# ThatRedox/ChunkyClPlugin

Hardware: NVIDIA B200
Metric: path samples/sec (higher is better)
Workload: dtype f32

## Files before the change

### chunkyclplugin_b200/csrc/ccu_device.cuh

```cuda
#pragma once
#include "ccu_math.cuh"

namespace ccu {

#define CCU_ANY_TYPE 0x7FFFFFFE

struct DScene {
    const int *__restrict__ tree;
    int depth;
    const unsigned *__restrict__ top;
    const unsigned *__restrict__ wide;
    int cell_level, top_log2;
    int use_wide;
    const unsigned *__restrict__ air_top;
    const unsigned *__restrict__ air_wide;
    const unsigned *__restrict__ air_bricks;
    int air_cell_level, air_top_log2;
    const int *__restrict__ block_palette;
    int block_palette_len;
    const int *__restrict__ quad_models;
    const int *__restrict__ aabb_models;
    const int *__restrict__ mat_palette;
    const int4 *__restrict__ block_rec;
    const int4 *__restrict__ mat_rec;
    const int4 *__restrict__ quad_rec;
    const int4 *__restrict__ aabb_rec;
    const int *__restrict__ world_bvh;
    const int *__restrict__ actor_bvh;
    const int *__restrict__ trigs;
    int world_bvh_empty, actor_bvh_empty;
    const int4 *__restrict__ world_rec;
    const int4 *__restrict__ actor_rec;
// ... 376 lines not shown
        lvl -= 2;
        e = __ldg(s.wide + (size_t)e * 64 + ((((bx >> lvl) & 3) << 4) | (((by >> lvl) & 3) << 2) | ((bz >> lvl) & 3)));
    }
    level = (e >> 26) & 31;
    unsigned v = e & CCU_WIDE_ANY;
    return v == CCU_WIDE_ANY ? CCU_ANY_TYPE : (int)v;
}

struct March {
    float3 o, d, inv;
    float t;
    float limit;
    int steps;
};

struct MarchStart { float3 inv; float t; int entered; };
static __device__ __noinline__ MarchStart march_begin_core(int depth, float3 origin, float3 direction) {
    MarchStart ms;
    ms.inv = f3(1.0f / direction.x, 1.0f / direction.y, 1.0f / direction.z);
    ms.t = 0;
    ms.entered = 1;
    int lx = f2i(floorf(origin.x)) >> depth, ly = f2i(floorf(origin.y)) >> depth, lz = f2i(floorf(origin.z)) >> depth;
    if ((lx | ly | lz) != 0) {
        float size = (float)(1 << depth);
        Box cube = {0, size, 0, size, 0, size};
        float dist = box_entry(cube, origin, ms.inv);
        if (is_nan(dist) || dist < 0) ms.entered = 0;
        else ms.t += dist + CCU_OFFSET;
    }
    return ms;
}
__device__ __forceinline__ bool march_begin(const DScene &s, March &m, float3 origin, float3 direction, float limit) {
    const MarchStart ms = march_begin_core(s.depth, origin, direction);
    m.o = origin;
    m.d = direction;
    m.inv = ms.inv;
    m.t = ms.t;
    m.limit = limit;
    m.steps = 0;
    return ms.entered != 0;
}

struct Cell {
    float3 pos, q;
    int bx, by, bz;
};
__device__ __forceinline__ Cell march_cell(const March &m) {
    Cell c;
    c.pos = m.o + m.d * m.t;
    c.q = c.pos + m.d * CCU_OFFSET;
    c.bx = f2i(floorf(c.q.x)); c.by = f2i(floorf(c.q.y)); c.bz = f2i(floorf(c.q.z));
    return c;
}
// ... 25 lines not shown
    if (data == 0) {
        march_exit(m, c, level);
        return 0;
    }
    if (march_block(s, m, data, level, surf, hit_t)) {
        hit_block = data;
        hit_node = node;
        hit_cell = c;
        return 1;
    }
    return 0;
}

__device__ __forceinline__ bool octree_intersect_ref(const DScene &s, float3 origin, float3 direction, Record &rec, HitInfo &hi) {
    March m;
    if (!march_begin(s, m, origin, direction, rec.distance)) return false;
    for (;;) {
        float t;
        int block, node;
        Cell cell;
        int r = march_step_ref(s, m, rec.surf, t, block, node, cell);
        if (r == 1) {
            rec.distance = t;
            rec.material = block;
            hi.node = node;
            hi.kind = 1;
            hi.bx = cell.bx; hi.by = cell.by; hi.bz = cell.bz;
            return true;
        }
        if (r == 2) return false;
    }
// ... 196 lines not shown
```

### chunkyclplugin_b200/csrc/ccu_host.h

```cpp
#pragma once
#include <cuda_runtime.h>

#include <algorithm>
#include <cstdint>
#include <cstring>
#include <memory>
#include <mutex>
#include <string>
#include <thread>
#include <utility>
#include <vector>

#include "../../include/chunkycu.h"
#include "ccu_device.cuh"

namespace ccu_host {

int fail(int code, const char *fmt, ...);
const char *last_error();

#define CU(call)                                                                                                          \
    do {                                                                                                                  \
        cudaError_t e_ = (call);                                                                                          \
        if (e_ != cudaSuccess)                                                                                            \
// ... 115 lines not shown
        return fail(rc, "%s", error.c_str());
    }
};

struct SceneInfo {
    int depth = 0, sky_res = 0;
    int world_root = 0, actor_root = 0, use_bvh2 = 0, use_air = 0, air_deep = 0;
    int world_bvh_empty = 1, actor_bvh_empty = 1;
    int cell_level = 0, top_log2 = 0, use_wide = 0, air_cell_level = 4, air_top_log2 = 0;
    int atlas_w = 0, atlas_h = 0, atlas_layers = 0;
    float sky_intensity = 0;
    int sun_host[6] = {0, 0, 0, 0, 0, 0};
    bool have_sun = false, have_atlas = false, have_sky = false;
    float3 su{}, sv{}, sw{};
    float sun_radius_cos = 0;
};

enum SceneArray { OCTREE, BLOCK_PALETTE, QUAD_MODELS, AABB_MODELS, MAT_PALETTE, TRIANGLES, WORLD_BVH, ACTOR_BVH, N_ARRAYS };
struct ArrayDesc {
    const char *setter;
    bool optional;
};
constexpr ArrayDesc ARRAY_DESC[N_ARRAYS] = {
    {"ccu_scene_set_octree", false},      {"ccu_scene_set_block_palette", false}, {"ccu_scene_set_quad_models", true},
    {"ccu_scene_set_aabb_models", true},  {"ccu_scene_set_material_palette", false}, {"ccu_scene_set_triangles", true},
    {"ccu_scene_set_world_bvh", true},    {"ccu_scene_set_actor_bvh", true},
};
struct PackedArray {
    DevBuf<int> dev;
    std::shared_ptr<const std::vector<int>> host;
// ... 47 lines not shown
    size_t accum_floats = 0;
    size_t accum_align = 256;
    int accum_active = 0;
    const float *window_base = nullptr;
    ccu_host::HostBuf<float> pinned;
    ccu_host::SeedRing seeds;
    ccu_host::DevBuf<int> fh_scratch;
    ccu_host::DevBuf<unsigned> work_counter;
    ccu_host::DevBuf<int> bvh_deep;
    int yield_below = 20;
    int q_refill_min = 8;
    int q_march_bias = 4;
    int q_shade_min = 0;
    int q_sticky_min = 0;
    int q_march_warps = 18;
    int window_spp = 0;
    int closed_spp = 0;
    bool target_live = false;
    ccu_render_params params = {256, 5, 13.0f, 0, 0};
    ccu_host::MergeJob merge;

    float last_ms = 0;
    bool timing_pending = false;
    int64_t launches = 0;
};

namespace ccu_host {
int start_readback(ccu_ctx *c, const float *src_dev, size_t lo, size_t hi, cudaStream_t stream);
int merge_readback(ccu_ctx *c, size_t lo, size_t hi, double *sample_buffer, double ds, double dp, double sinv, unsigned max_threads);
int replicate_scene(ccu_ctx *src, ccu_ctx *dst);
// ... 3 lines not shown
```

### chunkyclplugin_b200/csrc/ccu_layout.h

```cpp
#pragma once
#include <algorithm>
#include <cmath>
#include <cstdlib>
#include <cstring>
#include <thread>
#include <unordered_map>
#include <vector>

#include "ccu_device.cuh"
#include "ccu_march.cuh"

namespace {
struct WideLayout {
    std::vector<unsigned> top, wide;
    int cell_level = 0, top_log2 = 0;
    bool ok = true;
};

inline unsigned wide_leaf(int word, int level, bool &ok) {
    long long v = -(long long)word;
    unsigned val;
    if (v == 0x7FFFFFFELL) val = CCU_WIDE_ANY;
    else if (v >= 0 && v < (long long)CCU_WIDE_ANY) val = (unsigned)v;
    else { ok = false; val = 0; }
// ... 192 lines not shown
                const size_t c0 = (size_t)(dim * t / nt) * dim * dim, c1 = (size_t)(dim * (t + 1) / nt) * dim * dim;
                for (size_t c = c0; c < c1; c++)
                    if (!(b.top[c] & CCU_WIDE_LEAF)) b.top[c] += top_off;
                b.wide.insert(b.wide.end(), p.wide.begin(), p.wide.end());
                b.wide_level.insert(b.wide_level.end(), p.wide_level.begin(), p.wide_level.end());
                b.bricks.insert(b.bricks.end(), p.bricks.begin(), p.bricks.end());
            }
            if (b.wide.size() / 64 >= 0x1FFFFFFu || b.bricks.size() / 256 >= 0x7FFFFFu) b.ok = false;
        }
    }
    if (b.wide.empty()) b.wide.assign(64, air_leaf(1, 0));
    if (b.bricks.empty()) b.bricks.assign(256, 0u);
    return b;
}

struct BvhLayout {
    std::vector<int> rec;
    int root = 0;
    bool ok = true;
};
struct BvhStage {
    BvhLayout world, actor;
    std::vector<int> tris;
    std::unordered_map<int, int> leaf_at;
    bool ok = true;
    int leaf(const std::vector<int> &trigs, int prim, bool &valid) {
        auto [at, fresh] = leaf_at.try_emplace(prim, 0);
        if (!fresh) return at->second;
        if (prim < 0 || (size_t)prim >= trigs.size()) { valid = false; return 0; }
        const int count = trigs[(size_t)prim];
// ... 159 lines not shown
```

### chunkyclplugin_b200/csrc/ccu_march.cuh

```cuda
#pragma once
#include "ccu_device.cuh"

namespace ccu {

#define CCU_BRICK_UNIFORM 0xC0000000u

struct LeanRay {
    float3 o, d, inv, doff;
    float t, limit;
    int steps;
    int fmx, fmy, fmz;
};

__device__ __forceinline__ void lean_prepare(LeanRay &r) {
    r.doff = r.d * CCU_OFFSET;
    r.fmx = r.inv.x < 0.0f ? 0 : -1;
    r.fmy = r.inv.y < 0.0f ? 0 : -1;
    r.fmz = r.inv.z < 0.0f ? 0 : -1;
}

__device__ __forceinline__ float lean_exit_axis(int b, int low, int fm, float q, float inv) {
    const int plane = ((b & ~low) | (low & fm)) - fm;
    return fmaxf(((float)plane - q) * inv, -inff_());
}
// ... 56 lines not shown
    const int level = leaf ? ((int)(e << 1)) >> 27 : lvl_brick;
    const int low = (1 << (level & 31)) - 1;
    const float ex = lean_exit_axis(bx, low, r.fmx, q.x, r.inv.x);
    const float ey = lean_exit_axis(by, low, r.fmy, q.y, r.inv.y);
    const float ez = lean_exit_axis(bz, low, r.fmz, q.z, r.inv.z);
    const float tn = r.t + (fminf(ex, fminf(ey, ez)) + CCU_OFFSET);
    const bool adv = active && !fin && level >= 0;
    r.t = adv ? tn : r.t;
    r.steps += adv ? 1 : 0;
    return active ? (fin ? 2 : (level < 0 ? 1 : 0)) : done;
}

template <bool DEEP>
__device__ __forceinline__ bool octree_intersect_lean(const DScene &s, float3 origin, float3 direction, Record &rec, HitInfo &hi) {
    March m;
    if (!march_begin(s, m, origin, direction, rec.distance)) return false;
    LeanRay r;
    r.o = m.o; r.d = m.d; r.inv = m.inv; r.t = m.t; r.limit = m.limit; r.steps = m.steps;
    lean_prepare(r);
    for (;;) {
        const int st = lean_probe<DEEP, false>(s, s.air_top, r);
        if (st == 0) continue;
        if (st == 2) return false;
        m.t = r.t; m.steps = r.steps;
        const Cell c = march_cell(m);
        int level;
        const int data = find_leaf_wide(s, c.bx, c.by, c.bz, level);
        float t;
        if (march_block(s, m, data, level, rec.surf, t)) {
            rec.distance = t;
            rec.material = data;
// ... 79 lines not shown
```

### chunkyclplugin_b200/csrc/ccu_queue.cuh

```cuda
#pragma once
#include "ccu_march.cuh"

#ifndef CCU_Q_WARPS
#define CCU_Q_WARPS 28
#endif
#ifndef CCU_Q_ROWS
#define CCU_Q_ROWS 32
#endif

namespace ccu {

constexpr int Q_WARPS = CCU_Q_WARPS;
constexpr int Q_ROWS = CCU_Q_ROWS;
constexpr int Q_SLOTS = Q_ROWS * 32;
constexpr int Q_MW = (Q_ROWS + 31) / 32;
static_assert(Q_ROWS >= 1 && Q_ROWS <= 64, "at most two mask words per stage and column");

enum QStage : int { QS_MARCH = 0, QS_BLOCK, QS_EXIT, QS_END, QS_BVH, QS_SHADE, QS_LEAF, QS_COUNT_BVH };
constexpr int QS_COUNT = QS_BVH;

enum QField : int {
    QF_GID = 0, QF_META, QF_RNG, QF_COLX, QF_COLY, QF_COLZ, QF_THRX, QF_THRY, QF_THRZ,
    QF_SNX, QF_SNY, QF_SNZ, QF_SHW,
    QF_OX, QF_OY, QF_OZ, QF_DX, QF_DY, QF_DZ, QF_IX, QF_IY, QF_IZ, QF_T, QF_LIMIT, QF_STEPS,
// ... 172 lines not shown
        }
        do {
            if (LAY != 2) done = lean_step_flat<LAY == 0>(s, top, r, cur >= 0 && done == 0, done);
            else if (cur >= 0 && done == 0) done = lean_probe<LAY == 2, LAY == 0>(s, top, r);
            n_fly = __popc(__ballot_sync(full, cur >= 0 && done == 0));
            QSTAT(10, 1); QSTAT(11, n_fly);
        } while (busy - n_fly < refill_min && n_fly != 0);
    }
    if (cur >= 0) {
        F[QF_T * Q_SLOTS + cur] = __float_as_uint(r.t);
        F[QF_STEPS * Q_SLOTS + cur] = (uint32_t)r.steps;
        q_push(mask, done == 0 ? QS_MARCH : (done == 1 ? QS_BLOCK : QS_EXIT), cur & 31, cur >> 5);
    }
}

__device__ __forceinline__ void q_shade(const DScene &s, uint32_t *F, unsigned *mask, int lane, int row, float3 o, float3 d, float distance,
                                        bool ray_hit, const Surf &hit) {
    const int slot = row * 32 + lane;
    uint32_t meta = QU(QF_META) & ~QM_HIT;
    const bool shadow = (meta & QM_SHADOW) != 0;
    bool sun = false, bounce = false;
    float3 from = o;
    float3 normal = f3(0, 0, 0);
    if (!ray_hit) {
        float3 throughput = f3(QFL(QF_THRX), QFL(QF_THRY), QFL(QF_THRZ));
        float3 color = f3(QFL(QF_COLX), QFL(QF_COLY), QFL(QF_COLZ));
        float3 sky = sky_radiance(s, d);
        color = color + (sky * throughput) * (shadow ? QFL(QF_SHW) : 1.0f);
        QFL(QF_COLX) = color.x; QFL(QF_COLY) = color.y; QFL(QF_COLZ) = color.z;
        if (shadow) bounce = true;
// ... 33 lines not shown
        next_limit = distance;
    } else {
        next_d = diffuse_direction_sc(normal, x1, sn, cs);
        next_o = from + next_d * CCU_OFFSET;
        next_limit = inff_();
        const int ray_depth = (int)((meta >> 16) & 0xFF) + 1;
        meta = (meta & ~(0xFFu << 16) & ~QM_SHADOW) | ((uint32_t)ray_depth << 16);
        QU(QF_META) = meta;
        if (!(ray_depth < s.max_depth)) {
            next_ray = false;
            q_push(mask, QS_END, lane, row);
        }
    }
    if (next_ray) {
        March m;
        const bool entered = march_begin(s, m, next_o, next_d, next_limit);
        q_store_ray(F, mask, lane, row, m, entered);
    }
}

template <bool HAS_BVH>
__device__ __forceinline__ bool q_stage_resolve(const DScene &s, uint32_t *F, unsigned *mask, int lane, const bool kind_block, int min_lanes) {
    const int row = q_pop_batch(mask, kind_block ? QS_BLOCK : QS_EXIT, lane, min_lanes);
    if (row == -2) return false;
    QSTAT(2 * (kind_block ? QS_BLOCK : QS_EXIT), 1); QSTAT(2 * (kind_block ? QS_BLOCK : QS_EXIT) + 1, __popc(__ballot_sync(0xffffffffu, row >= 0)));
    if (row < 0) return true;
    const int slot = row * 32 + lane;
    March m;
    m.o = f3(QFL(QF_OX), QFL(QF_OY), QFL(QF_OZ));
    m.d = f3(QFL(QF_DX), QFL(QF_DY), QFL(QF_DZ));
    m.inv = f3(QFL(QF_IX), QFL(QF_IY), QFL(QF_IZ));
// ... 22 lines not shown
            QFL(QF_HNX) = hit.normal.x; QFL(QF_HNY) = hit.normal.y; QFL(QF_HNZ) = hit.normal.z;
            QFL(QF_HCX) = hit.color.x; QFL(QF_HCY) = hit.color.y; QFL(QF_HCZ) = hit.color.z;
        }
        const uint32_t meta = QU(QF_META);
        QU(QF_META) = ray_hit ? (meta | QM_HIT) : (meta & ~QM_HIT);
        if (ray_hit && (meta & QM_SHADOW)) {
            q_push(mask, QS_SHADE, lane, row);
            return true;
        }
        int ref, phase;
        bvh_first_ref(s, ref, phase);
        QI(QF_BREF) = ref;
        QI(QF_BSP) = phase << 8;
        q_push(mask, ref < 0 ? QS_LEAF : QS_BVH, lane, row);
    } else {
        q_shade(s, F, mask, lane, row, m.o, m.d, distance, ray_hit, hit);
    }
    return true;
}

__device__ __forceinline__ bool q_stage_shade(const DScene &s, uint32_t *F, unsigned *mask, int lane, int min_lanes) {
    const int row = q_pop_batch(mask, QS_SHADE, lane, min_lanes);
    if (row == -2) return false;
    QSTAT(22, 1); QSTAT(23, __popc(__ballot_sync(0xffffffffu, row >= 0)));
    if (row < 0) return true;
    const int slot = row * 32 + lane;
    const float3 o = f3(QFL(QF_OX), QFL(QF_OY), QFL(QF_OZ));
    const float3 d = f3(QFL(QF_DX), QFL(QF_DY), QFL(QF_DZ));
    const bool ray_hit = (QU(QF_META) & QM_HIT) != 0;
    Surf hit;
    hit.normal = f3(QFL(QF_HNX), QFL(QF_HNY), QFL(QF_HNZ));
    hit.color = make_float4(QFL(QF_HCX), QFL(QF_HCY), QFL(QF_HCZ), 0.0f);
    hit.emittance = QFL(QF_HEM);
    q_shade(s, F, mask, lane, row, o, d, QFL(QF_HDIST), ray_hit, hit);
    return true;
}

__device__ __forceinline__ float triangle_hit_aligned(const Int8 &q0, const int *__restrict__ t, float distance, float3 origin, float3 dir, float3 &normal,
                                                      float &ou, float &ov, int &material) {
    const int flags = q0.v[0];
    const float3 e1 = f3(i2f(q0.v[1]), i2f(q0.v[2]), i2f(q0.v[3]));
    const float3 e2 = f3(i2f(q0.v[4]), i2f(q0.v[5]), i2f(q0.v[6]));
    float3 pvec = cross3(dir, e2);
    float det = dot3(e1, pvec);
    if ((flags >> 8) & 1) {
        if (det > -CCU_EPS && det < CCU_EPS) return nanf_();
    } else if (det > -CCU_EPS) {
        return nanf_();
    }
// ... 192 lines not shown
    }
    if (PATCH && tw == Q_TILE_W && bh == Q_TILE_H) {
        ix = (in & 7u) | (((in >> 5) & 3u) << 3);
        iy = ((in >> 3) & 3u) | ((in >> 7) << 2);
    }
    py = band * Q_TILE_H + iy;
    px = tile * Q_TILE_W + ix;
}
template <bool PATCH = false>
__device__ __forceinline__ int tile_order_pixel(unsigned k, int W, int H) {
    unsigned px, py;
    tile_order_xy<PATCH>(k, W, H, px, py);
    return (int)(py * (unsigned)W + px);
}

template <bool LAST_FIRST>
__device__ __forceinline__ bool q_stage_end(const DScene &s, const PassParams &w, uint32_t *F, unsigned *mask, int *live, int lane, int min_lanes) {
    const unsigned full = 0xffffffffu;
    const int row = q_pop_batch(mask, QS_END, lane, min_lanes);
    if (row == -2) return false;
    QSTAT(2 * QS_END, 1); QSTAT(2 * QS_END + 1, __popc(__ballot_sync(full, row >= 0)));
    const int slot = row < 0 ? lane : row * 32 + lane;
    uint32_t meta = row >= 0 ? QU(QF_META) : 0u;
    int gid = row >= 0 ? QI(QF_GID) : 0;
    int pass = (int)(meta & 0xFFFFu);
    bool need_pixel = row >= 0 && (meta & QM_NEEDPIX) != 0;
    if (row >= 0 && !need_pixel) {
        float *px = w.res + (size_t)gid * 3;
        int spp = w.start_spp + pass;
        const float *pr = spp == 0 ? w.res_prev + (size_t)gid * 3 : px;
        float3 mean = f3(__ldcg(pr), __ldcg(pr + 1), __ldcg(pr + 2));
// ... 45 lines not shown
        }
    }
    const unsigned died = __ballot_sync(full, row >= 0 && !alive);
    if (died && lane == (__ffs((int)died) - 1)) atomicSub(live, __popc(died));
    if (!alive) return true;
    QI(QF_GID) = gid;
    QU(QF_META) = (uint32_t)pass;
    QFL(QF_COLX) = 0.0f; QFL(QF_COLY) = 0.0f; QFL(QF_COLZ) = 0.0f;
    QFL(QF_THRX) = 1.0f; QFL(QF_THRY) = 1.0f; QFL(QF_THRZ) = 1.0f;
    uint32_t rng = (uint32_t)__ldg(w.seeds + pass) + (uint32_t)gid;
    rng_next(rng);
    float3 o, d;
    camera_ray<false>(s, gid, rng, o, d);
    QU(QF_RNG) = rng;
    March m;
    const bool entered = march_begin(s, m, o, d, inff_());
    q_store_ray(F, mask, lane, row, m, entered);
    return true;
}

template <bool HAS_BVH, int LAY>
__global__ void __launch_bounds__(Q_WARPS * 32, 1) k_render_queue(const __grid_constant__ DScene s, const __grid_constant__ QueueParams qp) {
    constexpr int NST = q_stages(HAS_BVH);
    constexpr int MASK_WORDS = q_mask_words(HAS_BVH);
    extern __shared__ uint32_t q_mem[];
    uint32_t *F = q_mem;
    unsigned *mask = q_mem + q_fields(HAS_BVH) * Q_SLOTS;
    int *live = reinterpret_cast<int *>(mask + MASK_WORDS);
    unsigned *top_s = mask + MASK_WORDS + 32;
    int *stk = reinterpret_cast<int *>(top_s + (LAY == 0 ? Q_TOP_WORDS : 0));
    const unsigned full = 0xffffffffu;
// ... 47 lines not shown
            if (n > best_n) { best_n = n; best = st; }
        }
        }
        if (best < 0) {
            if (*reinterpret_cast<volatile int *>(live) == 0) break;
            QSTAT(12, 1);
            __nanosleep(100);
            continue;
        }
        const int min_lanes = held < 2 ? qp.shade_min : 1;
        bool ran = true;
        switch (best) {
            case QS_MARCH: QSTAT(0, 1); q_stage_march<NST, LAY>(s, top, F, mask, lane, qp.yield_below, qp.refill_min); break;
            case QS_BLOCK:
            case QS_EXIT: ran = q_stage_resolve<HAS_BVH>(s, F, mask, lane, best == QS_BLOCK, min_lanes); break;
            case QS_END: ran = q_stage_end<!HAS_BVH>(s, qp.w, F, mask, live, lane, min_lanes); break;
            case QS_BVH: QSTAT(16, 1); if (HAS_BVH) q_stage_bvh<NST>(s, F, mask, stk, qp.bvh_deep, lane, qp.yield_below, qp.refill_min); break;
            case QS_LEAF: if (HAS_BVH) ran = q_stage_leaf(s, F, mask, stk, qp.bvh_deep, lane, min_lanes); break;
            default: if (HAS_BVH) ran = q_stage_shade(s, F, mask, lane, min_lanes); break;
        }
        sticky = (ran && best != QS_MARCH && best != QS_BVH) ? best : -1;
        if (ran) {
            held = 0;
        } else {
            held++;
            __nanosleep(40);
        }
        __syncwarp();
    }
}

// ... 6 lines not shown
```

### chunkyclplugin_b200/csrc/chunkycu.cu

```cuda
#include <cuda_runtime.h>

#include <algorithm>
#include <cmath>
#include <cstdarg>
#include <cstdio>
#include <cstdlib>
#include <cstring>
#include <climits>
#include <mutex>
#include <string>
#include <thread>
#include <vector>

#include <chrono>

#include "ccu_host.h"
#include "ccu_march.cuh"
#include "ccu_queue.cuh"
#include "ccu_tonemap.cuh"
#include "ccu_layout.h"

using namespace ccu;


// ... 85 lines not shown
    uint32_t rng = (uint32_t)seed + (uint32_t)gid;
    rng_next(rng);
    float3 o, d;
    camera_ray_xy<false>(s, gid, (int)px, (int)py, rng, o, d);
    if (MODE == 0) {
        Record rec;
        rec.distance = inff_(); rec.material = 0; rec.surf.normal = f3(0, 0, 0); rec.point = f3(0, 0, 0);
        rec.surf.color = make_float4(0, 0, 0, 0); rec.surf.emittance = 0;
        HitInfo hi = {-1, 0, 0, 0, 0};
        bool hit = false;
        if (valid) hit = HAS_BVH ? closest_intersect_ref(s, o, d, rec, hi) : octree_intersect_ref(s, o, d, rec, hi);
        if (valid) first_hit_store(out, gid, hit, rec.material, rec.surf.normal, hi.node, hi.kind, rec.distance, rec.surf.color);
        return;
    }
    March m;
    const bool entered = march_begin(s, m, o, d, inff_());
    LeanRay r;
    r.o = m.o; r.d = m.d; r.inv = m.inv; r.t = m.t; r.limit = m.limit; r.steps = m.steps;
    lean_prepare(r);
    int st = (valid && entered) ? 0 : 2;
    Surf surf;
    surf.normal = f3(0, 0, 0); surf.color = make_float4(0, 0, 0, 0); surf.emittance = 0;
    float distance = inff_();
    int material = 0, hbx = 0, hby = 0, hbz = 0;
    for (;;) {
        st = first_hit_march<MODE == 2>(s, &r, st);
        if (st == 1) {
            m.t = r.t; m.steps = r.steps;
            const Cell c = march_cell(m);
            int level;
            const int data = find_leaf_wide(s, c.bx, c.by, c.bz, level);
// ... 142 lines not shown

int air_layout_id(const ccu_ctx *c) {
    if (c->scene.info.air_deep) return 2;
    return (c->scene.air_top.n <= (size_t)Q_TOP_WORDS && getenv("CCU_NO_TOPS") == nullptr) ? 0 : 1;
}

void fill_view(ccu_host::Scene &sc) {
    DScene &s = sc.view;
    const ccu_host::SceneInfo &in = sc.info;
    const auto arr = [&](ccu_host::SceneArray a) { return (const int *)sc.arrays[a].dev.p; };
    const auto rec = [](const DevBuf<int> &b) { return reinterpret_cast<const int4 *>(b.p); };
    s.tree = arr(ccu_host::OCTREE); s.depth = in.depth;
    s.top = sc.top.p; s.wide = sc.wide.p; s.cell_level = in.cell_level; s.top_log2 = in.top_log2; s.use_wide = in.use_wide;
    s.air_top = sc.air_top.p; s.air_wide = sc.air_wide.p; s.air_bricks = sc.air_bricks.p;
    s.air_cell_level = in.air_cell_level; s.air_top_log2 = in.air_top_log2;
    s.world_rec = rec(sc.world_rec); s.actor_rec = rec(sc.actor_rec); s.tris2 = sc.tris2.p;
    s.world_root = in.world_root; s.actor_root = in.actor_root;
    s.block_palette = arr(ccu_host::BLOCK_PALETTE); s.block_palette_len = (int)sc.arrays[ccu_host::BLOCK_PALETTE].dev.n;
    s.quad_models = arr(ccu_host::QUAD_MODELS); s.aabb_models = arr(ccu_host::AABB_MODELS); s.mat_palette = arr(ccu_host::MAT_PALETTE);
    s.block_rec = rec(sc.block_rec); s.mat_rec = rec(sc.mat_rec); s.quad_rec = rec(sc.quad_rec); s.aabb_rec = rec(sc.aabb_rec);
    s.world_bvh = arr(ccu_host::WORLD_BVH); s.actor_bvh = arr(ccu_host::ACTOR_BVH); s.trigs = arr(ccu_host::TRIANGLES);
    s.world_bvh_empty = in.world_bvh_empty; s.actor_bvh_empty = in.actor_bvh_empty;
    s.atlas = sc.atlas.p;
    s.atlas_w = in.atlas_w; s.atlas_h = in.atlas_h; s.atlas_layers = in.atlas_layers;
    s.atlas_tiles_x = (in.atlas_w + 15) / 16; s.atlas_tiles_y = (in.atlas_h + 15) / 16;
    s.sky = sc.sky.p; s.sky_res = in.sky_res; s.sky_intensity = in.sky_intensity;
    s.su = in.su; s.sv = in.sv; s.sw = in.sw; s.sun_radius_cos = in.sun_radius_cos;
    s.sun_flags = in.sun_host[0]; s.sun_tex_size = in.sun_host[1]; s.sun_tex = in.sun_host[2];
    memcpy(&s.sun_intensity, &in.sun_host[3], 4);
}

DScene launch_view(const ccu_ctx *c) {
    DScene s = c->scene.view;
    if (c->params.flags & CCU_RENDER_NO_ENTITIES) s.world_bvh_empty = s.actor_bvh_empty = 1;
    if (c->params.flags & CCU_RENDER_NO_SUN) s.sun_flags &= ~1;
    s.unorm = c->unorm.p;
    s.projector_type = c->projector_type;
    memcpy(s.cam, c->cam, sizeof s.cam);
    s.rays = c->rays[c->rays_active].p;
    s.width = c->width; s.height = c->height;
    s.half_width = (float)(c->width / (2.0 * c->height));
    s.inv_height = (float)(1.0 / c->height);
    s.draw_depth = c->params.draw_depth; s.max_depth = c->params.max_depth; s.emitter_scale = c->params.emitter_scale;
    return s;
// ... 193 lines not shown
    if (rc != CCU_OK) return rc;
    if (n == 0) return fail(CCU_ENODEVICE, "no CUDA device");
    if (device_index < 0 || device_index >= n) return fail(CCU_EINVAL, "device index %d out of range [0,%d)", device_index, n);
    cudaDeviceProp p;
    CU(cudaGetDeviceProperties(&p, device_index));
    if (p.major != 10) return fail(CCU_ENODEVICE, "device %d is sm_%d%d; this library is built for sm_100a only", device_index, p.major, p.minor);
    ccu_ctx *c = new ccu_ctx();
    c->device = device_index;
    c->sm_count = p.multiProcessorCount;
    if (const char *e = getenv("CCU_Q_MARCH_WARPS")) c->q_march_warps = std::max(1, std::min(64, atoi(e)));
    if (const char *e = getenv("CCU_Q_MARCH_BIAS")) c->q_march_bias = std::max(-32, std::min(32, atoi(e)));
    if (const char *e = getenv("CCU_Q_REFILL_MIN")) c->q_refill_min = std::max(1, std::min(32, atoi(e)));
    if (const char *e = getenv("CCU_Q_STICKY")) c->q_sticky_min = std::max(1, std::min(33, atoi(e)));
    if (const char *e = getenv("CCU_Q_SHADE_MIN")) c->q_shade_min = std::max(0, std::min(32, atoi(e)));
    if (const char *e = getenv("CCU_YIELD_BELOW")) c->yield_below = std::max(0, std::min(33, atoi(e)));
    DeviceGuard g(device_index);
    cudaError_t e = c->stream.create();
    if (e == cudaSuccess) e = c->copy_stream.create();
    if (e == cudaSuccess) e = c->ev0.create(cudaEventDefault);
    if (e == cudaSuccess) e = c->ev1.create(cudaEventDefault);
    if (e == cudaSuccess) e = c->window_ev.create(cudaEventDisableTiming);
    for (Event &ev : c->chunk_ev) if (e == cudaSuccess) e = ev.create(cudaEventDisableTiming);
    for (Event &ev : c->rays_used) if (e == cudaSuccess) e = ev.create(cudaEventDisableTiming);
    for (bool bvh : {false, true})
        for (int lay = 0; lay < 3 && e == cudaSuccess; lay++)
            e = cudaFuncSetAttribute(queue_kernel(bvh, lay), cudaFuncAttributeMaxDynamicSharedMemorySize, Q_SMEM_LIMIT);
    if (e == cudaSuccess) e = c->unorm.alloc(256);
    if (e == cudaSuccess) {
        k_unorm_table<<<1, 256, 0, c->stream>>>(c->unorm.p);
        c->launches++;
// ... 141 lines not shown
        const std::vector<int> &tree = host(ccu_host::OCTREE);
        WideLayout wl = build_wide_layout(tree.data(), tree.size(), in.depth);
        in.use_wide = (enable && wl.ok) ? 1 : 0;
        in.cell_level = wl.cell_level;
        in.top_log2 = wl.top_log2;
        CU(sc.top.upload(wl.top.data(), wl.top.size(), c->stream));
        CU(sc.wide.upload(wl.wide.data(), wl.wide.size(), c->stream));
        AirLayout al = build_air_layout(tree.data(), tree.size(), in.depth);
        in.use_air = (enable && al.ok) ? 1 : 0;
        in.air_cell_level = al.cell_level;
        in.air_top_log2 = al.top_log2;
        in.air_deep = al.cell_level > 4 ? 1 : 0;
        CU(sc.air_top.upload(al.top.data(), al.top.size(), c->stream));
        CU(sc.air_wide.upload(al.wide.data(), al.wide.size(), c->stream));
        CU(sc.air_bricks.upload(al.bricks.data(), al.bricks.size(), c->stream));
    }
    {
        PaletteRecs pr = build_palette_recs(host(ccu_host::BLOCK_PALETTE), host(ccu_host::MAT_PALETTE), host(ccu_host::QUAD_MODELS),
                                            host(ccu_host::AABB_MODELS));
        CU(sc.block_rec.upload(pr.block.data(), pr.block.size(), c->stream));
        CU(sc.mat_rec.upload(pr.mat.data(), pr.mat.size(), c->stream));
        CU(sc.quad_rec.upload(pr.quad.data(), pr.quad.size(), c->stream));
        CU(sc.aabb_rec.upload(pr.aabb.data(), pr.aabb.size(), c->stream));
    }
    {
        const std::vector<int> &world = host(ccu_host::WORLD_BVH), &actor = host(ccu_host::ACTOR_BVH);
        const BvhStage bs = build_bvh_stage(world, actor, host(ccu_host::TRIANGLES));
        in.world_bvh_empty = bvh_is_empty(world);
        in.actor_bvh_empty = bvh_is_empty(actor);
        in.use_bvh2 = bs.ok ? 1 : 0;
// ... 128 lines not shown
static int render_passes_locked(ccu_ctx *c, const int32_t *seeds, int32_t n_passes, bool first_chunk) {
    ccu_host::SeedRing &ring = c->seeds;
    if (!ring.dev.p) {
        ccu_host::SeedRing r;
        CU(r.dev.alloc((size_t)SEED_SLOTS * SEED_SLOT_INTS));
        CU(r.pinned.alloc((size_t)SEED_SLOTS * SEED_SLOT_INTS));
        for (Event &ev : r.ev) CU(ev.create(cudaEventDisableTiming));
        ring = std::move(r);
    }
    const int slot = ring.slot;
    ring.slot = (slot + 1) % SEED_SLOTS;
    CU(cudaEventSynchronize(ring.ev[slot]));
    int *seeds_host = ring.pinned + (size_t)slot * SEED_SLOT_INTS, *seeds_dev = ring.dev.p + (size_t)slot * SEED_SLOT_INTS;
    memcpy(seeds_host, seeds, (size_t)n_passes * sizeof(int));
    CU(cudaMemcpyAsync(seeds_dev, seeds_host, (size_t)n_passes * sizeof(int), cudaMemcpyHostToDevice, c->stream));
    const DScene s = launch_view(c);
    const int n_pixels = c->width * c->height;
    if (!c->work_counter.p) CU(c->work_counter.alloc(1));
    if (first_chunk) CU(cudaEventRecord(c->ev0, c->stream));
    const bool bvh = !(s.world_bvh_empty && s.actor_bvh_empty);
    const int mode = layout_mode(c);
    float *res = c->accum[c->accum_active].p;
    const float *res_prev = c->window_spp == 0 ? c->window_base : res;
    int kernel = c->params.kernel;
    if (kernel == 0) kernel = (mode != 0 && (!bvh || c->scene.info.use_bvh2)) ? 4 : 1;
    if (kernel == 1) {
        const int threads = 128, blocks = (n_pixels + threads - 1) / threads;
        dispatch<3>(mode, [&](auto M) {
            k_render_mega<M><<<blocks, threads, 0, c->stream>>>(s, seeds_dev, n_passes, c->window_spp, res, res_prev, n_pixels);
        });
    } else {
// ... 4 lines not shown
        qp.w.seeds = seeds_dev;
        qp.w.n_passes = n_passes;
        qp.w.start_spp = c->window_spp;
        qp.w.res = res;
        qp.w.res_prev = res_prev;
        qp.w.n_pixels = n_pixels;
        qp.w.next_pixel = c->work_counter.p;
        qp.yield_below = c->yield_below;
        qp.refill_min = c->q_refill_min;
        qp.march_bias = c->q_march_bias;
        qp.shade_min = c->q_shade_min;
        qp.sticky_min = c->q_sticky_min > 0 ? c->q_sticky_min : (bvh ? 16 : 33);
        qp.march_warps = bvh ? 64 : c->q_march_warps;
        const int lay = air_layout_id(c);
        const int grid = c->sm_count, block = Q_WARPS * 32;
        const int sky_texels = c->scene.info.sky_res * c->scene.info.sky_res;
        const int base_smem = q_smem_bytes(bvh, lay == 0);
        const char *sky_env = getenv("CCU_SKY_SMEM_MAX");
        const int sky_max = sky_env ? atoi(sky_env) : 16384;
        const bool sky_smem = sky_texels * 4 <= sky_max && base_smem + sky_texels * 4 <= Q_SMEM_LIMIT;
        qp.sky_texels = sky_smem ? sky_texels : 0;
        qp.bvh_deep = nullptr;
        if (bvh) {
            if (!c->bvh_deep.p) CU(c->bvh_deep.alloc((size_t)c->sm_count * Q_SLOTS * Q_DEEP));
            qp.bvh_deep = c->bvh_deep.p;
        }
        const int smem = base_smem + qp.sky_texels * 4;
        queue_kernel(bvh, lay)<<<grid, block, smem, c->stream>>>(s, qp);
#ifdef CCU_Q_STATS
        {
// ... 365 lines not shown
        return fail(CCU_EINVAL, "ccu_debug_bvh_layout: bad argument");
    const BvhStage s = build_bvh_stage(std::vector<int>(bvh, bvh + n_bvh), {}, std::vector<int>(trigs, trigs + n_trigs));
    const std::vector<int> &r = s.world.rec, &t = s.tris;
    *ok = s.ok ? 1 : 0;
    *root = s.world.root;
    *rec_words = (int64_t)r.size();
    *tris_words = (int64_t)t.size();
    if (rec) {
        if (rec_cap < (int64_t)r.size()) return fail(CCU_EINVAL, "ccu_debug_bvh_layout: rec buffer too small");
        std::copy(r.begin(), r.end(), rec);
    }
    if (tris) {
        if (tris_cap < (int64_t)t.size()) return fail(CCU_EINVAL, "ccu_debug_bvh_layout: tris buffer too small");
        std::copy(t.begin(), t.end(), tris);
    }
    return CCU_OK;
}

int ccu_debug_layout_lookup(const int32_t *tree, int64_t n, int32_t depth, const int32_t *xyz, int64_t count, int32_t *wide_value,
                            int32_t *wide_level, int32_t *air_solid, int32_t *air_level) {
    if (!tree || n < 1 || depth < 0 || depth > 30 || (count > 0 && !xyz)) return fail(CCU_EINVAL, "ccu_debug_layout_lookup: bad argument");
    WideLayout wl = build_wide_layout(tree, (size_t)n, depth);
    AirLayout al = build_air_layout(tree, (size_t)n, depth);
    if (!al.ok) return fail(CCU_ESTATE, "air layout could not be built");
    const int cl = wl.cell_level, tl = wl.top_log2;
    for (int64_t i = 0; i < count; i++) {
        const int bx = xyz[3 * i], by = xyz[3 * i + 1], bz = xyz[3 * i + 2];
        if (((bx | by | bz) >> depth) != 0) return fail(CCU_EINVAL, "voxel %lld outside the octree cube", (long long)i);
        if (wl.ok) {
            const size_t cell = ((((size_t)(bx >> cl) << tl) + (size_t)(by >> cl)) << tl) + (size_t)(bz >> cl);
// ... 37 lines not shown
```

### chunkyclplugin_b200/native.py

```python
from __future__ import annotations

import ctypes as C
import os
from typing import Optional

import numpy as np

_HERE = os.path.dirname(os.path.abspath(__file__))
LIB_PATH = os.environ.get("CHUNKYCU_LIB") or os.path.join(_HERE, "libchunkycu.so")

CCU_RENDER_NO_ENTITIES, CCU_RENDER_NO_SUN = 1, 2
CCU_UNIQUE_ID_BYTES = 128

CCU_OK, CCU_ENODEVICE, CCU_EINVAL, CCU_ECUDA, CCU_ENOMEM, CCU_ESTATE = 0, -1, -2, -3, -4, -5


class ChunkyCuError(RuntimeError):

    def __init__(self, code: int, message: str):
        super().__init__(f"[{code}] {message}")
        self.code = code


class RenderParams(C.Structure):
# ... 39 lines not shown
    "ccu_render_reset_window": (C.c_int, [_vp]),
    "ccu_render_set_window_spp": (C.c_int, [_vp, _i32]),
    "ccu_render_end": (C.c_int, [_vp]),
    "ccu_render_device_buffer": (C.c_int, [_vp, C.POINTER(_vp), C.POINTER(_i64)]),
    "ccu_render_scale": (C.c_int, [_vp, _f]),
    "ccu_stream_handle": (C.c_int, [_vp, C.POINTER(_vp)]),
    "ccu_first_hit": (C.c_int, [_vp, _i32, _vp, _vp, _vp, _vp, _vp, _vp, _vp]),
    "ccu_preview": (C.c_int, [_vp, _vp]),
    "ccu_last_kernel_ms": (C.c_int, [_vp, C.POINTER(_f)]),
    "ccu_launch_count": (C.c_int, [_vp, C.POINTER(_i64)]),
    "ccu_scene_device_bytes": (C.c_int, [_vp, C.POINTER(_i64)]),
    "ccu_scene_commit_ms": (C.c_int, [_vp, C.POINTER(C.c_double)]),
    "ccu_tonemap": (C.c_int, [_vp, _i32, _i32, _f, _vp, _i32, _vp]),
    "ccu_bench_gather": (C.c_int, [_vp, _i64, _i32, C.POINTER(_f), C.POINTER(_f)]),
    "ccu_debug_layout_lookup": (C.c_int, [_vp, _i64, _i32, _vp, _i64, _vp, _vp, _vp, _vp]),
    "ccu_debug_bvh_layout": (C.c_int, [_vp, _i64, _vp, _i64, _vp, _i64, _vp, _i64, C.POINTER(_i64), C.POINTER(_i64), _pi32, _pi32]),
    "ccu_group_create": (C.c_int, [_vp, _i32, C.POINTER(_vp)]),
    "ccu_group_unique_id": (C.c_int, [_vp]),
    "ccu_group_join": (C.c_int, [_vp, _vp, _i32, _i32, C.POINTER(_vp)]),
    "ccu_group_destroy": (C.c_int, [_vp]),
    "ccu_group_size": (C.c_int, [_vp, _pi32, _pi32]),
    "ccu_group_member": (C.c_int, [_vp, _i32, C.POINTER(_vp)]),
    "ccu_group_replicate_scene": (C.c_int, [_vp]),
    "ccu_group_camera_set": (C.c_int, [_vp, _i32, _vp, _i64]),
    "ccu_group_render_begin": (C.c_int, [_vp, _i32, _i32]),
    "ccu_group_render_set_params": (C.c_int, [_vp, C.POINTER(RenderParams)]),
    "ccu_group_render_passes": (C.c_int, [_vp, _vp, _i32]),
    "ccu_group_render_sync": (C.c_int, [_vp]),
    "ccu_group_render_merge": (C.c_int, [_vp, _vp, _i32, _pi32]),
    "ccu_group_render_merge_async": (C.c_int, [_vp, _vp, _i32, _pi32]),
# ... 43 lines not shown

def _ptr(a: Optional[np.ndarray]):
    return None if a is None else a.ctypes.data_as(C.c_void_p)


def layout_lookup(tree: np.ndarray, depth: int, xyz: np.ndarray):
    tree = np.ascontiguousarray(tree, dtype=np.int32)
    xyz = np.ascontiguousarray(xyz, dtype=np.int32).reshape(-1, 3)
    n = xyz.shape[0]
    out = {k: np.empty(n, dtype=np.int32) for k in ("wide_value", "wide_level", "air_solid", "air_level")}
    check(load().ccu_debug_layout_lookup(_ptr(tree), tree.size, depth, _ptr(xyz), n, _ptr(out["wide_value"]), _ptr(out["wide_level"]),
                                         _ptr(out["air_solid"]), _ptr(out["air_level"])))
    return out


def debug_bvh_layout(bvh: np.ndarray, trigs: np.ndarray):
    bvh = np.ascontiguousarray(bvh, dtype=np.int32)
    trigs = np.ascontiguousarray(trigs, dtype=np.int32)
    nr, nt, root, ok = _i64(), _i64(), _i32(), _i32()
    lib = load()
    check(lib.ccu_debug_bvh_layout(_ptr(bvh), bvh.size, _ptr(trigs), trigs.size, None, 0, None, 0, C.byref(nr), C.byref(nt), C.byref(root), C.byref(ok)))
    rec = np.zeros(max(nr.value, 1), dtype=np.int32)
    tris = np.zeros(max(nt.value, 1), dtype=np.int32)
    check(lib.ccu_debug_bvh_layout(_ptr(bvh), bvh.size, _ptr(trigs), trigs.size, _ptr(rec), rec.size, _ptr(tris), tris.size,
                                   C.byref(nr), C.byref(nt), C.byref(root), C.byref(ok)))
    return rec[:nr.value].reshape(-1, 16), tris[:nt.value], root.value, bool(ok.value)


def device_count() -> int:
    n = C.c_int()
# ... 310 lines not shown
```

### include/chunkycu.h

```cpp
#ifndef CHUNKYCU_H
#define CHUNKYCU_H

#include <stddef.h>
#include <stdint.h>

#ifdef __cplusplus
extern "C" {
#endif

#define CCU_OK 0
#define CCU_ENODEVICE (-1)
#define CCU_EINVAL (-2)
#define CCU_ECUDA (-3)
#define CCU_ENOMEM (-4)
#define CCU_ESTATE (-5)

typedef struct ccu_ctx ccu_ctx;

typedef struct ccu_render_params {
    int32_t draw_depth;
    int32_t max_depth;
    float emitter_scale;
    int32_t kernel;
    int32_t flags;
// ... 48 lines not shown

int ccu_first_hit(ccu_ctx *ctx, int32_t seed, int32_t *block, int32_t *face, int32_t *node, int32_t *kind, float *t,
                  float *normal, float *color);

int ccu_preview(ccu_ctx *ctx, int32_t *argb);

int ccu_tonemap(ccu_ctx *ctx, int32_t width, int32_t height, float exposure, const double *input, int32_t type, int32_t *argb);

int ccu_last_kernel_ms(ccu_ctx *ctx, float *ms);
int ccu_launch_count(ccu_ctx *ctx, int64_t *launches);
int ccu_scene_device_bytes(ccu_ctx *ctx, int64_t *bytes);
int ccu_scene_commit_ms(ccu_ctx *ctx, double *ms);
int ccu_bench_gather(ccu_ctx *ctx, int64_t array_bytes, int32_t dependent, float *gbytes_per_s, float *ns_per_load);
int ccu_debug_layout_lookup(const int32_t *tree, int64_t n, int32_t depth, const int32_t *xyz, int64_t count, int32_t *wide_value,
                            int32_t *wide_level, int32_t *air_solid, int32_t *air_level);

int ccu_debug_bvh_layout(const int32_t *bvh, int64_t n_bvh, const int32_t *trigs, int64_t n_trigs, int32_t *rec, int64_t rec_cap,
                         int32_t *tris, int64_t tris_cap, int64_t *rec_words, int64_t *tris_words, int32_t *root, int32_t *ok);

typedef struct ccu_group ccu_group;
#define CCU_UNIQUE_ID_BYTES 128
int ccu_group_create(const int32_t *devices, int32_t n, ccu_group **out);
int ccu_group_unique_id(uint8_t id[CCU_UNIQUE_ID_BYTES]);
int ccu_group_join(ccu_ctx *ctx, const uint8_t id[CCU_UNIQUE_ID_BYTES], int32_t rank, int32_t world, ccu_group **out);
int ccu_group_destroy(ccu_group *g);
int ccu_group_size(ccu_group *g, int32_t *world, int32_t *local_members);
int ccu_group_member(ccu_group *g, int32_t local_index, ccu_ctx **ctx);
int ccu_group_replicate_scene(ccu_group *g);
int ccu_group_camera_set(ccu_group *g, int32_t projector_type, const float *settings, int64_t n_floats);
int ccu_group_render_begin(ccu_group *g, int32_t width, int32_t height);
// ... 15 lines not shown
```

Measured before the change: 3.165 billion.

## Clip octree march limit to bounding box of non-empty voxels

Computes on the host a tight bounding box of all non-air octree nodes, padded by one voxel. At march start, each ray's limit is clipped to where it leaves this box, so rays stop marching through empty space outside the solid region. The clip applies to camera rays and to secondary rays in scenes without a BVH, and only when the box is at most a quarter of the octree volume. It adds a slab test per ray and a host tree walk at scene commit, and it relies on the limit clip being exact near boundaries.

```diff
diff --git a/chunkyclplugin_b200/csrc/ccu_device.cuh b/chunkyclplugin_b200/csrc/ccu_device.cuh
--- a/chunkyclplugin_b200/csrc/ccu_device.cuh
+++ b/chunkyclplugin_b200/csrc/ccu_device.cuh
@@ -16,6 +16,8 @@
     const unsigned *__restrict__ air_wide;
     const unsigned *__restrict__ air_bricks;
     int air_cell_level, air_top_log2;
+    float3 cut_lo, cut_hi;
+    float cut_reach;
     const int *__restrict__ block_palette;
     int block_palette_len;
     const int *__restrict__ quad_models;
@@ -422,8 +424,9 @@
     int steps;
 };
 
-struct MarchStart { float3 inv; float t; int entered; };
-static __device__ __noinline__ MarchStart march_begin_core(int depth, float3 origin, float3 direction) {
+struct MarchStart { float3 inv; float t, limit; int entered; };
+static __device__ __noinline__ MarchStart march_begin_core(int depth, float3 origin, float3 direction, float limit, float3 lo, float3 hi,
+                                                           float reach) {
     MarchStart ms;
     ms.inv = f3(1.0f / direction.x, 1.0f / direction.y, 1.0f / direction.z);
     ms.t = 0;
@@ -436,15 +439,28 @@
         if (is_nan(dist) || dist < 0) ms.entered = 0;
         else ms.t += dist + CCU_OFFSET;
     }
+    ms.limit = limit;
+    if (reach < 0.0f) return ms;
+    const float span = fabsf(origin.x) + fabsf(origin.y) + fabsf(origin.z) + fabsf(direction.x) + fabsf(direction.y) + fabsf(direction.z);
+    const float imax = fmaxf(fabsf(ms.inv.x), fmaxf(fabsf(ms.inv.y), fabsf(ms.inv.z)));
+    if (span <= reach && imax <= 0x1p64f) {
+        const float3 inv = ms.inv;
+        const float nx = ((inv.x >= 0.0f ? lo.x : hi.x) - origin.x) * inv.x, fx = ((inv.x >= 0.0f ? hi.x : lo.x) - origin.x) * inv.x;
+        const float ny = ((inv.y >= 0.0f ? lo.y : hi.y) - origin.y) * inv.y, fy = ((inv.y >= 0.0f ? hi.y : lo.y) - origin.y) * inv.y;
+        const float nz = ((inv.z >= 0.0f ? lo.z : hi.z) - origin.z) * inv.z, fz = ((inv.z >= 0.0f ? hi.z : lo.z) - origin.z) * inv.z;
+        const float enter = fmaxf(nx, fmaxf(ny, nz)), leave = fminf(fx, fminf(fy, fz));
+        ms.limit = fminf(limit, enter > leave ? -inff_() : leave);
+    }
     return ms;
 }
+template <bool CUT>
 __device__ __forceinline__ bool march_begin(const DScene &s, March &m, float3 origin, float3 direction, float limit) {
-    const MarchStart ms = march_begin_core(s.depth, origin, direction);
+    const MarchStart ms = march_begin_core(s.depth, origin, direction, limit, s.cut_lo, s.cut_hi, CUT ? s.cut_reach : -1.0f);
     m.o = origin;
     m.d = direction;
     m.inv = ms.inv;
     m.t = ms.t;
-    m.limit = limit;
+    m.limit = CUT ? ms.limit : limit;
     m.steps = 0;
     return ms.entered != 0;
 }
@@ -500,7 +516,7 @@
 
 __device__ __forceinline__ bool octree_intersect_ref(const DScene &s, float3 origin, float3 direction, Record &rec, HitInfo &hi) {
     March m;
-    if (!march_begin(s, m, origin, direction, rec.distance)) return false;
+    if (!march_begin<true>(s, m, origin, direction, rec.distance)) return false;
     for (;;) {
         float t;
         int block, node;
diff --git a/chunkyclplugin_b200/csrc/ccu_host.h b/chunkyclplugin_b200/csrc/ccu_host.h
--- a/chunkyclplugin_b200/csrc/ccu_host.h
+++ b/chunkyclplugin_b200/csrc/ccu_host.h
@@ -153,6 +153,7 @@
     bool have_sun = false, have_atlas = false, have_sky = false;
     float3 su{}, sv{}, sw{};
     float sun_radius_cos = 0;
+    int solid_lo[3] = {0, 0, 0}, solid_hi[3] = {0, 0, 0};
 };
 
 enum SceneArray { OCTREE, BLOCK_PALETTE, QUAD_MODELS, AABB_MODELS, MAT_PALETTE, TRIANGLES, WORLD_BVH, ACTOR_BVH, N_ARRAYS };
@@ -230,6 +231,7 @@
     int q_shade_min = 0;
     int q_sticky_min = 0;
     int q_march_warps = 18;
+    bool cube_cut = false;
     int window_spp = 0;
     int closed_spp = 0;
     bool target_live = false;
diff --git a/chunkyclplugin_b200/csrc/ccu_layout.h b/chunkyclplugin_b200/csrc/ccu_layout.h
--- a/chunkyclplugin_b200/csrc/ccu_layout.h
+++ b/chunkyclplugin_b200/csrc/ccu_layout.h
@@ -1,5 +1,6 @@
 #pragma once
 #include <algorithm>
+#include <climits>
 #include <cmath>
 #include <cstdlib>
 #include <cstring>
@@ -230,6 +231,45 @@
     return b;
 }
 
+struct SolidBox {
+    int lo[3] = {INT_MAX, INT_MAX, INT_MAX}, hi[3] = {INT_MIN, INT_MIN, INT_MIN};
+    size_t visits = 0;
+    bool covers(int x, int y, int z, int size) const {
+        return x >= lo[0] && y >= lo[1] && z >= lo[2] && x + size <= hi[0] && y + size <= hi[1] && z + size <= hi[2];
+    }
+    void add(int x, int y, int z, int size) {
+        const int p[3] = {x, y, z};
+        for (int i = 0; i < 3; i++) {
+            lo[i] = std::min(lo[i], p[i]);
+            hi[i] = std::max(hi[i], p[i] + size);
+        }
+    }
+};
+
+inline void solid_box_walk(const int *tree, size_t n, size_t idx, int level, int x, int y, int z, SolidBox &b) {
+    const int size = 1 << level;
+    const int w = tree[idx];
+    if (w == 0 || b.visits > n || b.covers(x, y, z, size)) return;
+    b.visits++;
+    if (w < 0 || level == 0 || (size_t)w + 7 >= n) { b.add(x, y, z, size); return; }
+    const int h = level - 1;
+    for (int c = 0; c < 8; c++)
+        solid_box_walk(tree, n, (size_t)w + c, h, x + (((c >> 2) & 1) << h), y + (((c >> 1) & 1) << h), z + ((c & 1) << h), b);
+}
+
+inline SolidBox solid_box(const int *tree, size_t n, int depth) {
+    SolidBox b;
+    solid_box_walk(tree, n, 0, depth, 0, 0, 0, b);
+    if (b.visits > n) {
+        b = SolidBox();
+        b.add(0, 0, 0, 1 << depth);
+    } else if (b.lo[0] > b.hi[0]) {
+        b = SolidBox();
+        for (int i = 0; i < 3; i++) b.lo[i] = b.hi[i] = 0;
+    }
+    return b;
+}
+
 struct BvhLayout {
     std::vector<int> rec;
     int root = 0;
diff --git a/chunkyclplugin_b200/csrc/ccu_march.cuh b/chunkyclplugin_b200/csrc/ccu_march.cuh
--- a/chunkyclplugin_b200/csrc/ccu_march.cuh
+++ b/chunkyclplugin_b200/csrc/ccu_march.cuh
@@ -94,7 +94,7 @@
 template <bool DEEP>
 __device__ __forceinline__ bool octree_intersect_lean(const DScene &s, float3 origin, float3 direction, Record &rec, HitInfo &hi) {
     March m;
-    if (!march_begin(s, m, origin, direction, rec.distance)) return false;
+    if (!march_begin<true>(s, m, origin, direction, rec.distance)) return false;
     LeanRay r;
     r.o = m.o; r.d = m.d; r.inv = m.inv; r.t = m.t; r.limit = m.limit; r.steps = m.steps;
     lean_prepare(r);
diff --git a/chunkyclplugin_b200/csrc/ccu_queue.cuh b/chunkyclplugin_b200/csrc/ccu_queue.cuh
--- a/chunkyclplugin_b200/csrc/ccu_queue.cuh
+++ b/chunkyclplugin_b200/csrc/ccu_queue.cuh
@@ -210,6 +210,7 @@
     }
 }
 
+template <bool HAS_BVH>
 __device__ __forceinline__ void q_shade(const DScene &s, uint32_t *F, unsigned *mask, int lane, int row, float3 o, float3 d, float distance,
                                         bool ray_hit, const Surf &hit) {
     const int slot = row * 32 + lane;
@@ -273,7 +274,7 @@
     }
     if (next_ray) {
         March m;
-        const bool entered = march_begin(s, m, next_o, next_d, next_limit);
+        const bool entered = march_begin<!HAS_BVH>(s, m, next_o, next_d, next_limit);
         q_store_ray(F, mask, lane, row, m, entered);
     }
 }
@@ -326,7 +327,7 @@
         QI(QF_BSP) = phase << 8;
         q_push(mask, ref < 0 ? QS_LEAF : QS_BVH, lane, row);
     } else {
-        q_shade(s, F, mask, lane, row, m.o, m.d, distance, ray_hit, hit);
+        q_shade<false>(s, F, mask, lane, row, m.o, m.d, distance, ray_hit, hit);
     }
     return true;
 }
@@ -344,7 +345,7 @@
     hit.normal = f3(QFL(QF_HNX), QFL(QF_HNY), QFL(QF_HNZ));
     hit.color = make_float4(QFL(QF_HCX), QFL(QF_HCY), QFL(QF_HCZ), 0.0f);
     hit.emittance = QFL(QF_HEM);
-    q_shade(s, F, mask, lane, row, o, d, QFL(QF_HDIST), ray_hit, hit);
+    q_shade<true>(s, F, mask, lane, row, o, d, QFL(QF_HDIST), ray_hit, hit);
     return true;
 }
 
@@ -567,7 +568,7 @@
     return (int)(py * (unsigned)W + px);
 }
 
-template <bool LAST_FIRST>
+template <bool LAST_FIRST, bool CUT>
 __device__ __forceinline__ bool q_stage_end(const DScene &s, const PassParams &w, uint32_t *F, unsigned *mask, int *live, int lane, int min_lanes) {
     const unsigned full = 0xffffffffu;
     const int row = q_pop_batch(mask, QS_END, lane, min_lanes);
@@ -643,7 +644,7 @@
     camera_ray<false>(s, gid, rng, o, d);
     QU(QF_RNG) = rng;
     March m;
-    const bool entered = march_begin(s, m, o, d, inff_());
+    const bool entered = march_begin<CUT>(s, m, o, d, inff_());
     q_store_ray(F, mask, lane, row, m, entered);
     return true;
 }
@@ -721,7 +722,7 @@
             case QS_MARCH: QSTAT(0, 1); q_stage_march<NST, LAY>(s, top, F, mask, lane, qp.yield_below, qp.refill_min); break;
             case QS_BLOCK:
             case QS_EXIT: ran = q_stage_resolve<HAS_BVH>(s, F, mask, lane, best == QS_BLOCK, min_lanes); break;
-            case QS_END: ran = q_stage_end<!HAS_BVH>(s, qp.w, F, mask, live, lane, min_lanes); break;
+            case QS_END: ran = q_stage_end<!HAS_BVH, !HAS_BVH>(s, qp.w, F, mask, live, lane, min_lanes); break;
             case QS_BVH: QSTAT(16, 1); if (HAS_BVH) q_stage_bvh<NST>(s, F, mask, stk, qp.bvh_deep, lane, qp.yield_below, qp.refill_min); break;
             case QS_LEAF: if (HAS_BVH) ran = q_stage_leaf(s, F, mask, stk, qp.bvh_deep, lane, min_lanes); break;
             default: if (HAS_BVH) ran = q_stage_shade(s, F, mask, lane, min_lanes); break;
diff --git a/chunkyclplugin_b200/csrc/chunkycu.cu b/chunkyclplugin_b200/csrc/chunkycu.cu
--- a/chunkyclplugin_b200/csrc/chunkycu.cu
+++ b/chunkyclplugin_b200/csrc/chunkycu.cu
@@ -123,7 +123,7 @@
         return;
     }
     March m;
-    const bool entered = march_begin(s, m, o, d, inff_());
+    const bool entered = march_begin<true>(s, m, o, d, inff_());
     LeanRay r;
     r.o = m.o; r.d = m.d; r.inv = m.inv; r.t = m.t; r.limit = m.limit; r.steps = m.steps;
     lean_prepare(r);
@@ -296,6 +296,10 @@
     s.top = sc.top.p; s.wide = sc.wide.p; s.cell_level = in.cell_level; s.top_log2 = in.top_log2; s.use_wide = in.use_wide;
     s.air_top = sc.air_top.p; s.air_wide = sc.air_wide.p; s.air_bricks = sc.air_bricks.p;
     s.air_cell_level = in.air_cell_level; s.air_top_log2 = in.air_top_log2;
+    const bool empty = in.solid_lo[0] >= in.solid_hi[0] || in.solid_lo[1] >= in.solid_hi[1] || in.solid_lo[2] >= in.solid_hi[2];
+    s.cut_lo = empty ? make_float3(1, 1, 1) : make_float3(in.solid_lo[0] - 1.0f, in.solid_lo[1] - 1.0f, in.solid_lo[2] - 1.0f);
+    s.cut_hi = empty ? make_float3(0, 0, 0) : make_float3(in.solid_hi[0] + 1.0f, in.solid_hi[1] + 1.0f, in.solid_hi[2] + 1.0f);
+    s.cut_reach = in.depth <= 19 ? (float)(4 << in.depth) : -1.0f;
     s.world_rec = rec(sc.world_rec); s.actor_rec = rec(sc.actor_rec); s.tris2 = sc.tris2.p;
     s.world_root = in.world_root; s.actor_root = in.actor_root;
     s.block_palette = arr(ccu_host::BLOCK_PALETTE); s.block_palette_len = (int)sc.arrays[ccu_host::BLOCK_PALETTE].dev.n;
@@ -310,6 +314,15 @@
     s.su = in.su; s.sv = in.sv; s.sw = in.sw; s.sun_radius_cos = in.sun_radius_cos;
     s.sun_flags = in.sun_host[0]; s.sun_tex_size = in.sun_host[1]; s.sun_tex = in.sun_host[2];
     memcpy(&s.sun_intensity, &in.sun_host[3], 4);
+}
+
+bool cut_pays_per_ray_start(const DScene &s) {
+    const double edge = (double)(1u << s.depth);
+    double vol = 1.0;
+    vol *= std::max(0.0, std::min((double)s.cut_hi.x, edge) - std::max((double)s.cut_lo.x, 0.0));
+    vol *= std::max(0.0, std::min((double)s.cut_hi.y, edge) - std::max((double)s.cut_lo.y, 0.0));
+    vol *= std::max(0.0, std::min((double)s.cut_hi.z, edge) - std::max((double)s.cut_lo.z, 0.0));
+    return s.cut_reach > 0 && vol * 4.0 <= edge * edge * edge;
 }
 
 DScene launch_view(const ccu_ctx *c) {
@@ -533,6 +546,7 @@
     if (const char *e = getenv("CCU_Q_STICKY")) c->q_sticky_min = std::max(1, std::min(33, atoi(e)));
     if (const char *e = getenv("CCU_Q_SHADE_MIN")) c->q_shade_min = std::max(0, std::min(32, atoi(e)));
     if (const char *e = getenv("CCU_YIELD_BELOW")) c->yield_below = std::max(0, std::min(33, atoi(e)));
+    c->cube_cut = getenv("CCU_NO_SOLID_BOX") != nullptr;
     DeviceGuard g(device_index);
     cudaError_t e = c->stream.create();
     if (e == cudaSuccess) e = c->copy_stream.create();
@@ -704,6 +718,11 @@
         CU(sc.air_top.upload(al.top.data(), al.top.size(), c->stream));
         CU(sc.air_wide.upload(al.wide.data(), al.wide.size(), c->stream));
         CU(sc.air_bricks.upload(al.bricks.data(), al.bricks.size(), c->stream));
+        SolidBox sb;
+        if (c->cube_cut) sb.add(0, 0, 0, 1 << in.depth);
+        else sb = solid_box(tree.data(), tree.size(), in.depth);
+        std::copy(sb.lo, sb.lo + 3, in.solid_lo);
+        std::copy(sb.hi, sb.hi + 3, in.solid_hi);
     }
     {
         PaletteRecs pr = build_palette_recs(host(ccu_host::BLOCK_PALETTE), host(ccu_host::MAT_PALETTE), host(ccu_host::QUAD_MODELS),
@@ -862,7 +881,7 @@
     int *seeds_host = ring.pinned + (size_t)slot * SEED_SLOT_INTS, *seeds_dev = ring.dev.p + (size_t)slot * SEED_SLOT_INTS;
     memcpy(seeds_host, seeds, (size_t)n_passes * sizeof(int));
     CU(cudaMemcpyAsync(seeds_dev, seeds_host, (size_t)n_passes * sizeof(int), cudaMemcpyHostToDevice, c->stream));
-    const DScene s = launch_view(c);
+    DScene s = launch_view(c);
     const int n_pixels = c->width * c->height;
     if (!c->work_counter.p) CU(c->work_counter.alloc(1));
     if (first_chunk) CU(cudaEventRecord(c->ev0, c->stream));
@@ -897,6 +916,7 @@
         qp.march_warps = bvh ? 64 : c->q_march_warps;
         const int lay = air_layout_id(c);
         const int grid = c->sm_count, block = Q_WARPS * 32;
+        if (!cut_pays_per_ray_start(c->scene.view)) s.cut_reach = -1.0f;
         const int sky_texels = c->scene.info.sky_res * c->scene.info.sky_res;
         const int base_smem = q_smem_bytes(bvh, lay == 0);
         const char *sky_env = getenv("CCU_SKY_SMEM_MAX");
@@ -1292,6 +1312,14 @@
         if (tris_cap < (int64_t)t.size()) return fail(CCU_EINVAL, "ccu_debug_bvh_layout: tris buffer too small");
         std::copy(t.begin(), t.end(), tris);
     }
+    return CCU_OK;
+}
+
+int ccu_debug_solid_box(const int32_t *tree, int64_t n, int32_t depth, int32_t *lo, int32_t *hi) {
+    if (!tree || n < 1 || depth < 0 || depth > 30 || !lo || !hi) return fail(CCU_EINVAL, "ccu_debug_solid_box: bad argument");
+    const SolidBox b = solid_box(tree, (size_t)n, depth);
+    std::copy(b.lo, b.lo + 3, lo);
+    std::copy(b.hi, b.hi + 3, hi);
     return CCU_OK;
 }
 
diff --git a/chunkyclplugin_b200/native.py b/chunkyclplugin_b200/native.py
--- a/chunkyclplugin_b200/native.py
+++ b/chunkyclplugin_b200/native.py
@@ -77,6 +77,7 @@
     "ccu_tonemap": (C.c_int, [_vp, _i32, _i32, _f, _vp, _i32, _vp]),
     "ccu_bench_gather": (C.c_int, [_vp, _i64, _i32, C.POINTER(_f), C.POINTER(_f)]),
     "ccu_debug_layout_lookup": (C.c_int, [_vp, _i64, _i32, _vp, _i64, _vp, _vp, _vp, _vp]),
+    "ccu_debug_solid_box": (C.c_int, [_vp, _i64, _i32, _pi32, _pi32]),
     "ccu_debug_bvh_layout": (C.c_int, [_vp, _i64, _vp, _i64, _vp, _i64, _vp, _i64, C.POINTER(_i64), C.POINTER(_i64), _pi32, _pi32]),
     "ccu_group_create": (C.c_int, [_vp, _i32, C.POINTER(_vp)]),
     "ccu_group_unique_id": (C.c_int, [_vp]),
@@ -150,6 +151,13 @@
     return out
 
 
+def debug_solid_box(tree: np.ndarray, depth: int):
+    tree = np.ascontiguousarray(tree, dtype=np.int32)
+    lo, hi = (_i32 * 3)(), (_i32 * 3)()
+    check(load().ccu_debug_solid_box(_ptr(tree), tree.size, depth, lo, hi))
+    return tuple(lo), tuple(hi)
+
+
 def debug_bvh_layout(bvh: np.ndarray, trigs: np.ndarray):
     bvh = np.ascontiguousarray(bvh, dtype=np.int32)
     trigs = np.ascontiguousarray(trigs, dtype=np.int32)
diff --git a/include/chunkycu.h b/include/chunkycu.h
--- a/include/chunkycu.h
+++ b/include/chunkycu.h
@@ -86,6 +86,7 @@
 int ccu_bench_gather(ccu_ctx *ctx, int64_t array_bytes, int32_t dependent, float *gbytes_per_s, float *ns_per_load);
 int ccu_debug_layout_lookup(const int32_t *tree, int64_t n, int32_t depth, const int32_t *xyz, int64_t count, int32_t *wide_value,
                             int32_t *wide_level, int32_t *air_solid, int32_t *air_level);
+int ccu_debug_solid_box(const int32_t *tree, int64_t n, int32_t depth, int32_t *lo, int32_t *hi);
 
 int ccu_debug_bvh_layout(const int32_t *bvh, int64_t n_bvh, const int32_t *trigs, int64_t n_trigs, int32_t *rec, int64_t rec_cap,
                          int32_t *tris, int64_t tris_cap, int64_t *rec_words, int64_t *tris_words, int32_t *root, int32_t *ok);
```

Result: slower. 3.095 billion (median of 6 runs) (-2.2%).
